# dcharatan/pixelsplat

Measured on NVIDIA H100. Metric: rendered views/sec fwd+bwd @256x256, 3 gauss/px, higher is better.
Workload: dtype f32

## Files before the change

### pixelsplat_b200/csrc/ps_common.cuh

```cuda
#pragma once
#include <cuda_runtime.h>
#include <stdint.h>

#include "../../include/pixelsplat_b200.h"

namespace ps {

constexpr int kTile = PS_TILE;
constexpr int kTilePixels = kTile * kTile;

struct Geom {
    float *depth;
    int32_t *radii;
    float2 *xy;
    float4 *conic_opacity;
    float4 *rgb;
    ushort4 *rect;
    uint8_t *clamped;
    uint32_t *tile_count;
    uint32_t *tile_start;
    uint32_t *tile_cursor;
    long long *n_instances;
    uint32_t *vis_pairs;
    uint32_t *vis_any;
    float4 *cull;
};

struct ImageState {
    float *final_T;
    uint32_t *n_contrib;
    float *color;
    float4 *run_state;
    float *depth_image;
    float *run_depth;
};

constexpr int kLossSlots = PS_LOSS_SLOTS;
struct LossEpilogue {
    const float *target;
    float *sums;
    const float *grad_scale;
};

constexpr int kMaxSegments = 4;

struct HitLists {
    uint2 *hits;
    uint32_t *run_hits;
};

struct Dims {
    int S, V, P, M, deg, sh_layout, cov_layout, H, W, gx, gy, tiles, sh_basis, segK, hit_lists;
    int depth_mode;
    long long capacity;
};

struct Inputs {
    const float *means, *cov, *opac, *sh, *view, *proj, *campos, *tanfov, *bg, *scale;
    const float *near_far;
};

struct ViewGrads {
    float2 *d_mean2d;
    float4 *d_conic;
    float4 *d_color;
};

constexpr float kDepthEps = 1e-10f;

__device__ __forceinline__ float depth_value(int mode, float vz, const float *scale, const float *near_far, int vid) {
    const float z = scale ? vz / scale[vid] : vz;
    if (mode == PS_DEPTH_DISPARITY) return 1.0f / z;
    if (mode == PS_DEPTH_RELATIVE_DISPARITY) {
        const float dn = 1.0f / (near_far[2 * vid] + kDepthEps), df = 1.0f / (near_far[2 * vid + 1] + kDepthEps);
        return 1.0f - (1.0f / (z + kDepthEps) - df) / (dn - df + kDepthEps);
    }
    if (mode == PS_DEPTH_LOG) return logf(fmaxf(fminf(z, near_far[2 * vid]), near_far[2 * vid + 1]));
    return z;
}

__device__ __forceinline__ float depth_value_grad(int mode, float vz, const float *scale, const float *near_far, int vid) {
    const float z = scale ? vz / scale[vid] : vz;
    if (mode == PS_DEPTH_DISPARITY) return -1.0f / (z * z);
    if (mode == PS_DEPTH_RELATIVE_DISPARITY) {
        const float dn = 1.0f / (near_far[2 * vid] + kDepthEps), df = 1.0f / (near_far[2 * vid + 1] + kDepthEps);
        const float iz = 1.0f / (z + kDepthEps);
        return iz * iz / (dn - df + kDepthEps);
    }
    if (mode == PS_DEPTH_LOG) {
        const float nr = near_far[2 * vid], fr = near_far[2 * vid + 1];
        const float m = fminf(z, nr);
        const float gm = z < nr ? 1.0f : (z == nr ? 0.5f : 0.0f);
        const float gr = m > fr ? 1.0f : (m == fr ? 0.5f : 0.0f);
        return gm * gr / fmaxf(m, fr);
    }
    return 1.0f;
}

__device__ __forceinline__ float2 cull_extent(float a, float c, float o) {
    if (!(a > 0.0f) || !(c > 0.0f) || !(o <= 3.0e38f)) return make_float2(3.0e38f, 3.0e38f);
    if (!(o * 255.0f >= 1.0f - 1e-3f)) return make_float2(-3.0e38f, -3.0e38f);
    const float tau2 = 2.0f * (__logf(fmaxf(o * 255.0f, 1.0f)) + 0.01f);
    return make_float2(sqrtf(tau2 * a) * 1.001f + 0.01f, sqrtf(tau2 * c) * 1.001f + 0.01f);
}

void set_error(const char *fmt, ...);

enum Mark { kMarkFwdStart = 0, kMarkPreprocess, kMarkScatter, kMarkSort, kMarkCompositeFwd,
            kMarkBwdStart, kMarkBwdZero, kMarkCompositeBwd, kMarkPreprocessBwd, kNumMarks };
void mark(int id, cudaStream_t st);
void count_launch();

bool first_use_on_device(unsigned long long &mask);

#define PS_CUDA_CHECK(expr)                                                              \
    do {                                                                                 \
        cudaError_t _e = (expr);                                                         \
        if (_e != cudaSuccess) {                                                         \
            ps::set_error("%s failed: %s (%s:%d)", #expr, cudaGetErrorString(_e), __FILE__, __LINE__); \
            return PS_ERR_CUDA;                                                          \
        }                                                                                \
    } while (0)

#define PS_LAUNCH_CHECK(name)                                                            \
    do {                                                                                 \
        cudaError_t _e = cudaGetLastError();                                             \
        if (_e != cudaSuccess) {                                                         \
            ps::set_error("launch of %s failed: %s", name, cudaGetErrorString(_e));      \
            return PS_ERR_CUDA;                                                          \
        }                                                                                \
        ps::count_launch();                                                              \
    } while (0)

int launch_preprocess(const Dims &d, const Inputs &in, const Geom &g, cudaStream_t st);
int launch_sh_color(const Dims &d, const Inputs &in, const Geom &g, cudaStream_t st);
int launch_binning(const Dims &d, const Geom &g, unsigned long long *keys,
                   unsigned long long *keys_alt, int sort_impl, int segment_hint, cudaStream_t st);
int launch_composite_forward(const Dims &d, const Inputs &in, const Geom &g,
                             const unsigned long long *keys, const ImageState &img,
                             float *out_color, const LossEpilogue &loss, const HitLists &hl, cudaStream_t st);
int launch_composite_backward(const Dims &d, const Inputs &in, const Geom &g,
                              const unsigned long long *keys, const ImageState &img,
                              const float *d_color, const float *d_depth, const ViewGrads &vg,
                              const LossEpilogue &loss, const HitLists &hl, cudaStream_t st);
int launch_composite_forward_v1(const Dims &d, const Inputs &in, const Geom &g,
                                const unsigned long long *keys, const ImageState &img,
                                float *out_color, cudaStream_t st);
int launch_composite_backward_v1(const Dims &d, const Inputs &in, const Geom &g,
                                 const unsigned long long *keys, const ImageState &img,
                                 const float *d_color, const ViewGrads &vg, cudaStream_t st);
int composite_impl();
int set_composite_option(int which, int value);
int get_composite_option(int which);
int composite_segments(long long tasks);
bool composite_hit_lists(long long capacity);
int launch_preprocess_backward(const Dims &d, const Inputs &in, const Geom &g, const ViewGrads &vg,
                               const ps_raster_grads &out, cudaStream_t st);
int launch_gradient_fill(const Dims &d, const ps_raster_grads &out, cudaStream_t st);

}
```

### pixelsplat_b200/csrc/raster_api.cu

```cuda
#include <cstdarg>
#include <atomic>
#include <cstdio>
#include <cstring>
#include <mutex>

#include "ps_common.cuh"

namespace ps {

static thread_local char g_error[512] = "";

void set_error(const char *fmt, ...) {
    va_list ap;
    va_start(ap, fmt);
    vsnprintf(g_error, sizeof(g_error), fmt, ap);
    va_end(ap);
}

static bool g_timing = false;
static cudaEvent_t g_events[kNumMarks];
static bool g_events_ready = false;
static std::atomic<unsigned long long> g_launches{0};

void count_launch() { g_launches.fetch_add(1, std::memory_order_relaxed); }

static std::mutex g_once_mutex;

bool first_use_on_device(unsigned long long &mask) {
    int dev = 0;
    cudaGetDevice(&dev);
    const unsigned long long bit = 1ull << (dev & 63);
    std::lock_guard<std::mutex> lock(g_once_mutex);
    if (mask & bit) return false;
    mask |= bit;
    return true;
}

void mark(int id, cudaStream_t st) {
    if (!g_timing) return;
    if (!g_events_ready) {
        for (int i = 0; i < kNumMarks; ++i) cudaEventCreate(&g_events[i]);
        g_events_ready = true;
    }
    cudaEventRecord(g_events[id], st);
}

struct SideCtx {
    cudaStream_t side = nullptr;
    cudaEvent_t fork = nullptr, join = nullptr;
    std::mutex enqueue;
};
static SideCtx g_side_ctx[64];

static int side_ready(SideCtx *&ctx) {
    int dev = 0;
    PS_CUDA_CHECK(cudaGetDevice(&dev));
    ctx = &g_side_ctx[dev & 63];
    std::lock_guard<std::mutex> lock(g_once_mutex);
    if (ctx->side) return PS_OK;
    PS_CUDA_CHECK(cudaStreamCreateWithFlags(&ctx->side, cudaStreamNonBlocking));
    PS_CUDA_CHECK(cudaEventCreateWithFlags(&ctx->fork, cudaEventDisableTiming));
    PS_CUDA_CHECK(cudaEventCreateWithFlags(&ctx->join, cudaEventDisableTiming));
    return PS_OK;
}

static size_t align_up(size_t x) { return (x + 255) & ~(size_t)255; }

struct Layout {
    ps_raster_layout off;
    ps_raster_sizes sizes;
};

static int validate(const ps_raster_desc *d) {
    if (!d) { set_error("desc is NULL"); return PS_ERR_INVALID_ARGUMENT; }
    if (d->n_scenes < 1 || d->views_per_scene < 1 || d->n_gaussians < 1) {
        set_error("n_scenes, views_per_scene and n_gaussians must be >= 1 (got %d, %d, %d)",
                  d->n_scenes, d->views_per_scene, d->n_gaussians);
        return PS_ERR_INVALID_ARGUMENT;
    }
    if (d->height < 1 || d->width < 1) { set_error("bad image size %dx%d", d->height, d->width); return PS_ERR_INVALID_ARGUMENT; }
    if (d->sh_coeffs < 0 || d->sh_coeffs > 25) { set_error("sh_coeffs must be in [0, 25], got %d", d->sh_coeffs); return PS_ERR_INVALID_ARGUMENT; }
    if (d->sh_degree < 0 || d->sh_degree > 4) { set_error("sh_degree must be in [0, 4], got %d", d->sh_degree); return PS_ERR_INVALID_ARGUMENT; }
    if (d->sh_coeffs > 0 && (d->sh_degree + 1) * (d->sh_degree + 1) > d->sh_coeffs) {
        set_error("sh_degree %d needs %d coefficients, only %d given", d->sh_degree,
                  (d->sh_degree + 1) * (d->sh_degree + 1), d->sh_coeffs);
        return PS_ERR_INVALID_ARGUMENT;
    }
    if (d->sh_layout != PS_SH_M3 && d->sh_layout != PS_SH_3M) { set_error("bad sh_layout %d", d->sh_layout); return PS_ERR_INVALID_ARGUMENT; }
    if (d->sh_basis != PS_SH_BASIS_3DGS && d->sh_basis != PS_SH_BASIS_E3NN) { set_error("bad sh_basis %d", d->sh_basis); return PS_ERR_INVALID_ARGUMENT; }
    if (d->depth_mode < PS_DEPTH_NONE || d->depth_mode > PS_DEPTH_LOG) { set_error("bad depth_mode %d (PS_DEPTH_*: 0..4)", d->depth_mode); return PS_ERR_INVALID_ARGUMENT; }
    if (d->cov_layout != PS_COV_TRIU6 && d->cov_layout != PS_COV_3X3) { set_error("bad cov_layout %d", d->cov_layout); return PS_ERR_INVALID_ARGUMENT; }
    if (d->instance_capacity < 1 || d->instance_capacity > 0x7fffffffll) {
        set_error("instance_capacity must be in [1, 2^31-1], got %lld", (long long)d->instance_capacity);
        return PS_ERR_INVALID_ARGUMENT;
    }
    const long long gx = (d->width + kTile - 1) / kTile, gy = (d->height + kTile - 1) / kTile;
    if (gx > 65535 || gy > 65535) { set_error("image too large for 16-bit tile rectangles"); return PS_ERR_UNSUPPORTED; }
    const long long segs = (long long)d->n_scenes * d->views_per_scene * gx * gy;
    if ((long long)d->n_scenes * d->views_per_scene * d->n_gaussians > 0xffffffffll) {
        set_error("scenes * views * gaussians must fit 32 bits");
        return PS_ERR_UNSUPPORTED;
    }
    if (segs > 0x7fffffffll || (long long)d->n_scenes * d->views_per_scene > 65535) {
        set_error("too many (view, tile) segments: %lld", segs);
        return PS_ERR_UNSUPPORTED;
    }
    return PS_OK;
}

static Dims make_dims(const ps_raster_desc *d) {
    Dims r;
    r.S = d->n_scenes; r.V = d->views_per_scene; r.P = d->n_gaussians; r.M = d->sh_coeffs;
    r.deg = d->sh_degree; r.sh_layout = d->sh_layout; r.cov_layout = d->cov_layout;
    r.H = d->height; r.W = d->width;
    r.gx = (d->width + kTile - 1) / kTile; r.gy = (d->height + kTile - 1) / kTile;
    r.tiles = r.gx * r.gy;
    r.capacity = d->instance_capacity;
    r.sh_basis = d->sh_basis;
    r.segK = composite_segments((long long)r.S * r.V * r.tiles * 8);
    r.hit_lists = composite_hit_lists(r.capacity) ? 1 : 0;
    r.depth_mode = d->depth_mode;
    return r;
}

static Layout make_layout(const ps_raster_desc *d) {
    const Dims m = make_dims(d);
    const size_t vp = (size_t)m.S * m.V * m.P;
    const size_t vt = (size_t)m.S * m.V * m.tiles;
    const size_t px = (size_t)m.S * m.V * m.H * m.W;
    Layout L;
    size_t o = 0;
    auto take = [&](size_t bytes) { const size_t at = o; o = align_up(o + bytes); return at; };
    L.off.depth = take(vp * 4);
    L.off.radii = take(vp * 4);
    L.off.xy = take(vp * 8);
    L.off.conic_opacity = take(vp * 16);
    L.off.rgb = take(vp * 16);
    L.off.rect = take(vp * 8);
    L.off.clamped = take(vp);
    L.off.tile_count = take(vt * 4);
    L.off.tile_start = take(vt * 4);
    L.off.tile_cursor = take(vt * 4);
    L.off.n_instances = take(32);
    L.off.vis_pairs = take(vp * 4);
    L.off.vis_any = take((size_t)m.S * m.P * 4);
    L.off.cull = take(vp * 16);
    L.sizes.geom_bytes = o;
    o = 0;
    L.off.keys = take((size_t)m.capacity * 8);
    L.off.keys_alt = take((size_t)m.capacity * 8);
    L.off.block_hits = L.off.run_hits = 0;
    if (m.hit_lists) {
        L.off.block_hits = take((size_t)m.capacity * 8 * 8);
        L.off.run_hits = take((size_t)m.S * m.V * m.tiles * 8 * kMaxSegments * 4);
    }
    L.sizes.binning_bytes = o;
    o = 0;
    L.off.final_T = take(px * 4);
    L.off.n_contrib = take(px * 4);
    L.off.color = take(px * 12);
    L.off.run_state = take(px * 16 * (kMaxSegments - 1));
    L.off.depth_image = L.off.run_depth = 0;
    if (m.depth_mode) {
        L.off.depth_image = take(px * 4);
        L.off.run_depth = take(px * 4 * (kMaxSegments - 1));
    }
    L.sizes.image_bytes = o;
    L.sizes.backward_bytes = align_up(vp * 8) + align_up(vp * 16) + align_up(vp * 16);
    return L;
}

static Geom make_geom(const Layout &L, void *geom) {
    char *b = static_cast<char *>(geom);
    Geom g;
    g.depth = reinterpret_cast<float *>(b + L.off.depth);
    g.radii = reinterpret_cast<int32_t *>(b + L.off.radii);
    g.xy = reinterpret_cast<float2 *>(b + L.off.xy);
    g.conic_opacity = reinterpret_cast<float4 *>(b + L.off.conic_opacity);
    g.rgb = reinterpret_cast<float4 *>(b + L.off.rgb);
    g.rect = reinterpret_cast<ushort4 *>(b + L.off.rect);
    g.clamped = reinterpret_cast<uint8_t *>(b + L.off.clamped);
    g.tile_count = reinterpret_cast<uint32_t *>(b + L.off.tile_count);
    g.tile_start = reinterpret_cast<uint32_t *>(b + L.off.tile_start);
    g.tile_cursor = reinterpret_cast<uint32_t *>(b + L.off.tile_cursor);
    g.n_instances = reinterpret_cast<long long *>(b + L.off.n_instances);
    g.vis_pairs = reinterpret_cast<uint32_t *>(b + L.off.vis_pairs);
    g.vis_any = reinterpret_cast<uint32_t *>(b + L.off.vis_any);
    g.cull = reinterpret_cast<float4 *>(b + L.off.cull);
    return g;
}

static ImageState make_image(const Layout &L, void *image) {
    char *b = static_cast<char *>(image);
    ImageState im;
    im.final_T = reinterpret_cast<float *>(b + L.off.final_T);
    im.n_contrib = reinterpret_cast<uint32_t *>(b + L.off.n_contrib);
    im.color = reinterpret_cast<float *>(b + L.off.color);
    im.run_state = reinterpret_cast<float4 *>(b + L.off.run_state);
    im.depth_image = L.off.depth_image ? reinterpret_cast<float *>(b + L.off.depth_image) : nullptr;
    im.run_depth = L.off.run_depth ? reinterpret_cast<float *>(b + L.off.run_depth) : nullptr;
    return im;
}

static int check_common(const ps_raster_desc *desc, const ps_raster_inputs *in, const ps_raster_state *state,
                        const Layout &L) {
    if (!in || !state) { set_error("inputs/state is NULL"); return PS_ERR_INVALID_ARGUMENT; }
    if (!in->means || !in->cov || !in->opacities || !in->sh || !in->viewmatrix || !in->projmatrix ||
        !in->campos || !in->tanfov || !in->background) {
        set_error("a required input pointer is NULL");
        return PS_ERR_INVALID_ARGUMENT;
    }
    if (!state->geom || !state->binning || !state->image) { set_error("a state buffer is NULL"); return PS_ERR_INVALID_ARGUMENT; }
    if (state->geom_bytes < L.sizes.geom_bytes || state->binning_bytes < L.sizes.binning_bytes ||
        state->image_bytes < L.sizes.image_bytes) {
        set_error("state buffers too small: need geom %zu binning %zu image %zu, got %zu %zu %zu",
                  L.sizes.geom_bytes, L.sizes.binning_bytes, L.sizes.image_bytes, state->geom_bytes,
                  state->binning_bytes, state->image_bytes);
        return PS_ERR_INVALID_ARGUMENT;
    }
    if (((uintptr_t)state->geom | (uintptr_t)state->binning | (uintptr_t)state->image) & 15) {
        set_error("state buffers must be 16-byte aligned");
        return PS_ERR_INVALID_ARGUMENT;
    }
    if ((desc->depth_mode == PS_DEPTH_RELATIVE_DISPARITY || desc->depth_mode == PS_DEPTH_LOG) && !in->near_far) {
        set_error("depth_mode %d needs ps_raster_inputs.near_far", desc->depth_mode);
        return PS_ERR_INVALID_ARGUMENT;
    }
    if (desc->depth_mode && composite_impl() == 1) {
        set_error("the legacy compositor (composite_impl = 1) has no depth channel");
        return PS_ERR_UNSUPPORTED;
    }
    return PS_OK;
}

static Inputs make_inputs(const ps_raster_inputs *in) {
    Inputs r;
    r.means = in->means; r.cov = in->cov; r.opac = in->opacities; r.sh = in->sh;
    r.view = in->viewmatrix; r.proj = in->projmatrix; r.campos = in->campos; r.tanfov = in->tanfov;
    r.bg = in->background; r.scale = in->scene_scale; r.near_far = in->near_far;
    return r;
}

}

using namespace ps;

extern "C" {

PS_API int ps_version(void) { return 100; }

PS_API const char *ps_last_error(void) { return g_error; }

PS_API unsigned long long ps_launch_count(void) { return g_launches.load(std::memory_order_relaxed); }

PS_API void ps_timing_enable(int on) { g_timing = on != 0; }

PS_API int ps_timing_read(float *ms) {
    if (!g_timing || !g_events_ready) { set_error("timing is not enabled"); return PS_ERR_INVALID_ARGUMENT; }
    static const int pairs[7][2] = {{kMarkFwdStart, kMarkPreprocess}, {kMarkPreprocess, kMarkScatter},
                                    {kMarkScatter, kMarkSort}, {kMarkSort, kMarkCompositeFwd},
                                    {kMarkBwdStart, kMarkBwdZero}, {kMarkBwdZero, kMarkCompositeBwd},
                                    {kMarkCompositeBwd, kMarkPreprocessBwd}};
    PS_CUDA_CHECK(cudaEventSynchronize(g_events[kMarkPreprocessBwd]));
    for (int i = 0; i < 7; ++i) PS_CUDA_CHECK(cudaEventElapsedTime(&ms[i], g_events[pairs[i][0]], g_events[pairs[i][1]]));
    return PS_OK;
}

PS_API int ps_set_option(const char *name, int value) {
    if (!name) { set_error("ps_set_option: name is NULL"); return PS_ERR_INVALID_ARGUMENT; }
    int rc = PS_ERR_INVALID_ARGUMENT;
    if (!strcmp(name, "composite_impl")) rc = set_composite_option(0, value);
    else if (!strcmp(name, "composite_segments")) rc = set_composite_option(1, value);
    else if (!strcmp(name, "composite_hit_lists")) rc = set_composite_option(2, value);
    if (rc) set_error("ps_set_option: unknown option or bad value: %s = %d", name, value);
    return rc;
}

PS_API int ps_get_option(const char *name, int *value) {
    if (!name || !value) { set_error("ps_get_option: name / value is NULL"); return PS_ERR_INVALID_ARGUMENT; }
    int which = -1;
    if (!strcmp(name, "composite_impl")) which = 0;
    else if (!strcmp(name, "composite_segments")) which = 1;
    else if (!strcmp(name, "composite_hit_lists")) which = 2;
    if (which < 0) { set_error("ps_get_option: unknown option %s", name); return PS_ERR_INVALID_ARGUMENT; }
    *value = get_composite_option(which);
    return PS_OK;
}

PS_API int ps_raster_sizes_query(const ps_raster_desc *desc, ps_raster_sizes *out) {
    int rc = validate(desc);
    if (rc) return rc;
    if (!out) { set_error("out is NULL"); return PS_ERR_INVALID_ARGUMENT; }
    *out = make_layout(desc).sizes;
    return PS_OK;
}

PS_API int ps_raster_layout_query(const ps_raster_desc *desc, ps_raster_layout *out) {
    int rc = validate(desc);
    if (rc) return rc;
    if (!out) { set_error("out is NULL"); return PS_ERR_INVALID_ARGUMENT; }
    *out = make_layout(desc).off;
    return PS_OK;
}

}

static int raster_forward_impl(const ps_raster_desc *desc, const ps_raster_inputs *in, const ps_raster_state *state,
                               float *out_color, int32_t *out_radii, int64_t *n_instances_host,
                               const ps_raster_loss *loss, void *stream) {
    int rc = validate(desc);
    if (rc) return rc;
    const Layout L = make_layout(desc);
    rc = check_common(desc, in, state, L);
    if (rc) return rc;
    LossEpilogue le{nullptr, nullptr, nullptr};
    if (loss) {
        if (!loss->target || !loss->sums) { set_error("ps_raster_loss: target / sums is NULL"); return PS_ERR_INVALID_ARGUMENT; }
        le.target = loss->target; le.sums = loss->sums;
    } else if (!out_color) {
        set_error("out_color is NULL");
        return PS_ERR_INVALID_ARGUMENT;
    }
    cudaStream_t st = static_cast<cudaStream_t>(stream);
    const Dims d = make_dims(desc);
    const Inputs I = make_inputs(in);
    const Geom g = make_geom(L, state->geom);
    unsigned long long *keys = reinterpret_cast<unsigned long long *>(static_cast<char *>(state->binning) + L.off.keys);
    unsigned long long *keys_alt = reinterpret_cast<unsigned long long *>(static_cast<char *>(state->binning) + L.off.keys_alt);
    const ImageState img = make_image(L, state->image);

    SideCtx *sc = nullptr;
    if ((rc = side_ready(sc))) return rc;
    std::lock_guard<std::mutex> enqueue_lock(sc->enqueue);
    mark(kMarkFwdStart, st);
    if ((rc = launch_preprocess(d, I, g, st))) return rc;
    mark(kMarkPreprocess, st);
    PS_CUDA_CHECK(cudaEventRecord(sc->fork, st));
    PS_CUDA_CHECK(cudaStreamWaitEvent(sc->side, sc->fork, 0));
    if ((rc = launch_sh_color(d, I, g, sc->side))) return rc;
    PS_CUDA_CHECK(cudaEventRecord(sc->join, sc->side));
    if ((rc = launch_binning(d, g, keys, keys_alt, desc->sort_impl, desc->sort_segment_hint, st))) return rc;
    mark(kMarkSort, st);
    PS_CUDA_CHECK(cudaStreamWaitEvent(st, sc->join, 0));
    if (n_instances_host)
        PS_CUDA_CHECK(cudaMemcpyAsync(n_instances_host, g.n_instances, 2 * sizeof(int64_t), cudaMemcpyDeviceToHost, st));
    if (le.sums)
        PS_CUDA_CHECK(cudaMemsetAsync(le.sums, 0, sizeof(float) * 2 * kLossSlots * (size_t)d.S * d.V, st));
    HitLists hl{nullptr, nullptr};
    if (d.hit_lists) {
        hl.hits = reinterpret_cast<uint2 *>(static_cast<char *>(state->binning) + L.off.block_hits);
        hl.run_hits = reinterpret_cast<uint32_t *>(static_cast<char *>(state->binning) + L.off.run_hits);
    }
    if ((rc = launch_composite_forward(d, I, g, keys, img, out_color, le, hl, st))) return rc;
    mark(kMarkCompositeFwd, st);
    if (out_radii)
        PS_CUDA_CHECK(cudaMemcpyAsync(out_radii, g.radii, sizeof(int32_t) * (size_t)d.S * d.V * d.P,
                                      cudaMemcpyDeviceToDevice, st));
    return PS_OK;
}

extern "C" {

PS_API int ps_raster_forward(const ps_raster_desc *desc, const ps_raster_inputs *in, const ps_raster_state *state,
                             float *out_color, int32_t *out_radii, int64_t *n_instances_host, void *stream) {
    return raster_forward_impl(desc, in, state, out_color, out_radii, n_instances_host, nullptr, stream);
}

PS_API int ps_raster_forward_loss(const ps_raster_desc *desc, const ps_raster_inputs *in, const ps_raster_state *state,
                                  const ps_raster_loss *loss, float *out_color, int32_t *out_radii,
                                  int64_t *n_instances_host, void *stream) {
    if (!loss) { set_error("ps_raster_forward_loss: loss is NULL"); return PS_ERR_INVALID_ARGUMENT; }
    return raster_forward_impl(desc, in, state, out_color, out_radii, n_instances_host, loss, stream);
}

}

static int raster_backward_impl(const ps_raster_desc *desc, const ps_raster_inputs *in, const ps_raster_state *state,
                                const float *d_color, const float *target, const float *grad_scale,
                                const float *d_depth, void *scratch, size_t scratch_bytes,
                                const ps_raster_grads *grads, void *stream) {
    int rc = validate(desc);
    if (rc) return rc;
    const Layout L = make_layout(desc);
    rc = check_common(desc, in, state, L);
    if (rc) return rc;
    if ((!d_color && !(target && grad_scale)) || !scratch || !grads) {
        set_error("d_color (or target + grad_scale) / scratch / grads is NULL");
        return PS_ERR_INVALID_ARGUMENT;
    }
    const LossEpilogue le{d_color ? nullptr : target, nullptr, d_color ? nullptr : grad_scale};
    if (!grads->d_means || !grads->d_cov || !grads->d_opacities || !grads->d_sh) {
        set_error("a required gradient pointer is NULL");
        return PS_ERR_INVALID_ARGUMENT;
    }
    if (scratch_bytes < L.sizes.backward_bytes || ((uintptr_t)scratch & 15)) {
        set_error("backward scratch too small or misaligned: need %zu, got %zu", L.sizes.backward_bytes, scratch_bytes);
        return PS_ERR_INVALID_ARGUMENT;
    }
    cudaStream_t st = static_cast<cudaStream_t>(stream);
    Dims d = make_dims(desc);
    if (!d_depth) d.depth_mode = 0;
    const Inputs I = make_inputs(in);
    const Geom g = make_geom(L, state->geom);
    const unsigned long long *keys = reinterpret_cast<const unsigned long long *>(static_cast<char *>(state->binning) + L.off.keys);
    const ImageState img = make_image(L, state->image);
    const size_t vp = (size_t)d.S * d.V * d.P;
    char *sb = static_cast<char *>(scratch);
    ViewGrads vg;
    vg.d_mean2d = reinterpret_cast<float2 *>(sb);
    vg.d_conic = reinterpret_cast<float4 *>(sb + align_up(vp * 8));
    vg.d_color = reinterpret_cast<float4 *>(sb + align_up(vp * 8) + align_up(vp * 16));
    SideCtx *sc = nullptr;
    if ((rc = side_ready(sc))) return rc;
    std::lock_guard<std::mutex> enqueue_lock(sc->enqueue);
    mark(kMarkBwdStart, st);
    PS_CUDA_CHECK(cudaEventRecord(sc->fork, st));
    PS_CUDA_CHECK(cudaStreamWaitEvent(sc->side, sc->fork, 0));
    if ((rc = launch_gradient_fill(d, *grads, sc->side))) return rc;
    PS_CUDA_CHECK(cudaEventRecord(sc->join, sc->side));
    PS_CUDA_CHECK(cudaMemsetAsync(scratch, 0, L.sizes.backward_bytes, st));
    mark(kMarkBwdZero, st);
    HitLists hl{nullptr, nullptr};
    if (d.hit_lists) {
        hl.hits = reinterpret_cast<uint2 *>(static_cast<char *>(state->binning) + L.off.block_hits);
        hl.run_hits = reinterpret_cast<uint32_t *>(static_cast<char *>(state->binning) + L.off.run_hits);
    }
    if ((rc = launch_composite_backward(d, I, g, keys, img, d_color, d_depth, vg, le, hl, st))) return rc;
    mark(kMarkCompositeBwd, st);
    PS_CUDA_CHECK(cudaStreamWaitEvent(st, sc->join, 0));
    if ((rc = launch_preprocess_backward(d, I, g, vg, *grads, st))) return rc;
    mark(kMarkPreprocessBwd, st);
    return PS_OK;
}

extern "C" {

PS_API int ps_raster_backward(const ps_raster_desc *desc, const ps_raster_inputs *in, const ps_raster_state *state,
                              const float *d_color, void *scratch, size_t scratch_bytes,
                              const ps_raster_grads *grads, void *stream) {
    if (!d_color) { set_error("d_color is NULL"); return PS_ERR_INVALID_ARGUMENT; }
    return raster_backward_impl(desc, in, state, d_color, nullptr, nullptr, nullptr, scratch, scratch_bytes, grads,
                                stream);
}

PS_API int ps_raster_backward_loss(const ps_raster_desc *desc, const ps_raster_inputs *in, const ps_raster_state *state,
                                   const float *target, const float *grad_scale, void *scratch, size_t scratch_bytes,
                                   const ps_raster_grads *grads, void *stream) {
    if (!target || !grad_scale) { set_error("target / grad_scale is NULL"); return PS_ERR_INVALID_ARGUMENT; }
    return raster_backward_impl(desc, in, state, nullptr, target, grad_scale, nullptr, scratch, scratch_bytes, grads,
                                stream);
}

PS_API int ps_raster_backward_depth(const ps_raster_desc *desc, const ps_raster_inputs *in, const ps_raster_state *state,
                                    const float *d_color, const float *loss_target, const float *grad_scale,
                                    const float *d_depth, void *scratch, size_t scratch_bytes,
                                    const ps_raster_grads *grads, void *stream) {
    if (!d_depth) { set_error("d_depth is NULL"); return PS_ERR_INVALID_ARGUMENT; }
    if (desc && desc->depth_mode == PS_DEPTH_NONE) {
        set_error("ps_raster_backward_depth needs the depth_mode of a depth forward (got 0)");
        return PS_ERR_INVALID_ARGUMENT;
    }
    if (!d_color && !(loss_target && grad_scale)) { set_error("d_color, or loss_target + grad_scale, is NULL"); return PS_ERR_INVALID_ARGUMENT; }
    return raster_backward_impl(desc, in, state, d_color, d_color ? nullptr : loss_target, d_color ? nullptr : grad_scale,
                                d_depth, scratch, scratch_bytes, grads, stream);
}

}
```

### pixelsplat_b200/csrc/raster_binning.cu

```cuda
#include <cub/device/device_segmented_radix_sort.cuh>

#include "ps_common.cuh"

namespace ps {

constexpr int kScanThreads = 1024;

__global__ void __launch_bounds__(kScanThreads)
k_tile_scan(int n, const uint32_t *__restrict__ count, uint32_t *__restrict__ start,
            uint32_t *__restrict__ cursor, long long *__restrict__ n_instances) {
    __shared__ uint32_t warp_sums[32];
    __shared__ unsigned long long carry_s;
    const int tid = threadIdx.x, lane = tid & 31, warp = tid >> 5;
    if (tid == 0) carry_s = 0;
    __syncthreads();
    uint32_t cmax = 0;
    for (int base = 0; base < n; base += kScanThreads) {
        const int i = base + tid;
        const uint32_t c = i < n ? count[i] : 0u;
        cmax = max(cmax, c);
        uint32_t x = c;
#pragma unroll
        for (int o = 1; o < 32; o <<= 1) {
            const uint32_t y = __shfl_up_sync(0xffffffffu, x, o);
            if (lane >= o) x += y;
        }
        if (lane == 31) warp_sums[warp] = x;
        __syncthreads();
        if (warp == 0) {
            uint32_t w = warp_sums[lane];
#pragma unroll
            for (int o = 1; o < 32; o <<= 1) {
                const uint32_t y = __shfl_up_sync(0xffffffffu, w, o);
                if (lane >= o) w += y;
            }
            warp_sums[lane] = w;
        }
        __syncthreads();
        const unsigned long long carry = carry_s;
        const uint32_t warp_off = warp ? warp_sums[warp - 1] : 0u;
        const unsigned long long excl = carry + warp_off + (x - c);
        if (i < n) {
            const uint32_t e = excl > 0xffffffffull ? 0xffffffffu : (uint32_t)excl;
            start[i] = e;
            cursor[i] = e;
        }
        __syncthreads();
        if (tid == kScanThreads - 1) carry_s = carry + warp_sums[31];
        __syncthreads();
    }
    if (tid == 0) *n_instances = (long long)carry_s;
    cmax = __reduce_max_sync(0xffffffffu, cmax);
    if (lane == 0 && cmax) atomicMax(reinterpret_cast<unsigned long long *>(n_instances + 1), (unsigned long long)cmax);
}

constexpr int kScatterThreads = 256;
constexpr int kScatterMaxSmemTiles = 8192;

__global__ void __launch_bounds__(kScatterThreads)
k_scatter(Dims d, Geom geo, unsigned long long *__restrict__ keys, int use_smem) {
    extern __shared__ uint32_t s_scatter[];
    if (*geo.n_instances > d.capacity) return;
    const int vid = blockIdx.y;
    const int g = blockIdx.x * kScatterThreads + threadIdx.x;
    uint32_t *cnt = s_scatter, *base = s_scatter + d.tiles;
    uint32_t *cur = geo.tile_cursor + (size_t)vid * d.tiles;
    const size_t vg = (size_t)vid * d.P + g;
    const bool vis = g < d.P && geo.radii[vg] > 0;
    ushort4 r = make_ushort4(0, 0, 0, 0);
    unsigned long long key = 0;
    if (vis) {
        r = geo.rect[vg];
        key = ((unsigned long long)__float_as_uint(geo.depth[vg]) << 32) | (uint32_t)g;
    }
    if (!use_smem) {
        for (int ty = r.y; ty < r.w; ++ty)
            for (int tx = r.x; tx < r.z; ++tx) keys[atomicAdd(&cur[ty * d.gx + tx], 1u)] = key;
        return;
    }
    for (int i = threadIdx.x; i < d.tiles; i += kScatterThreads) cnt[i] = 0;
    __syncthreads();
    for (int ty = r.y; ty < r.w; ++ty)
        for (int tx = r.x; tx < r.z; ++tx) atomicAdd(&cnt[ty * d.gx + tx], 1u);
    __syncthreads();
    for (int i = threadIdx.x; i < d.tiles; i += kScatterThreads) {
        const uint32_t c = cnt[i];
        if (c) { base[i] = atomicAdd(&cur[i], c); cnt[i] = 0; }
    }
    __syncthreads();
    for (int ty = r.y; ty < r.w; ++ty)
        for (int tx = r.x; tx < r.z; ++tx) {
            const int t = ty * d.gx + tx;
            keys[base[t] + atomicAdd(&cnt[t], 1u)] = key;
        }
}

template <int THREADS>
__device__ void bitonic_sort_smem(unsigned long long *s_keys, int n_pad) {
    constexpr int kWarps = THREADS / 32;
    const int lane = threadIdx.x & 31, warp = threadIdx.x >> 5;
    const int chunk = max(n_pad / kWarps, 2);
    const int warps_used = n_pad / chunk;
    const int half = n_pad >> 1;
    for (int k = 2; k <= n_pad; k <<= 1) {
        int j = k >> 1;
        const bool had_global = j >= chunk;
        for (; j >= chunk; j >>= 1) {
            for (int t = threadIdx.x; t < half; t += THREADS) {
                const int i = 2 * t - (t & (j - 1));
                const int p = i + j;
                const unsigned long long a = s_keys[i], b = s_keys[p];
                const bool up = (i & k) == 0;
                if ((a > b) == up) { s_keys[i] = b; s_keys[p] = a; }
            }
            __syncthreads();
        }
        if (warp < warps_used) {
            const int base = warp * chunk;
            for (; j > 0; j >>= 1) {
                for (int t = lane; t < (chunk >> 1); t += 32) {
                    const int i = base + 2 * t - (t & (j - 1));
                    const int p = i + j;
                    const unsigned long long a = s_keys[i], b = s_keys[p];
                    const bool up = (i & k) == 0;
                    if ((a > b) == up) { s_keys[i] = b; s_keys[p] = a; }
                }
                __syncwarp();
            }
        }
        if (had_global || 2 * k > chunk) __syncthreads();
    }
}

constexpr int kSortThreads = 512;
constexpr int kSortWarps = kSortThreads / 32;

struct SortSmem {
    uint32_t cnt[kSortWarps * 256];
    uint32_t misc[64];
};

__device__ unsigned long long *radix8_passes(unsigned long long *a, unsigned long long *b, int n, SortSmem &sm,
                                             int key_shift, uint32_t sub, int num_passes) {
    const int tid = threadIdx.x, lane = tid & 31, warp = tid >> 5;
    const int lo = (int)(((long long)n * warp) / kSortWarps);
    const int hi = (int)(((long long)n * (warp + 1)) / kSortWarps);
    uint32_t *cnt = sm.cnt, *misc = sm.misc;
    for (int p = 0; p < num_passes; ++p) {
        const int shift = 8 * p;
        auto digit = [&](unsigned long long k) -> uint32_t {
            return ((((uint32_t)(k >> key_shift)) - sub) >> shift) & 255u;
        };
        for (int i = tid; i < kSortWarps * 256; i += kSortThreads) cnt[i] = 0;
        if (tid == 0) misc[0] = 0;
        __syncthreads();
        for (int i = lo + lane; i < hi; i += 32) atomicAdd(&cnt[warp * 256 + digit(a[i])], 1u);
        __syncthreads();
        uint32_t total = 0, incl = 0;
        if (tid < 256) {
            uint32_t c[kSortWarps];
#pragma unroll
            for (int w = 0; w < kSortWarps; ++w) c[w] = cnt[w * 256 + tid];
#pragma unroll
            for (int w = 0; w < kSortWarps; ++w) { const uint32_t t = c[w]; c[w] = total; total += t; }
            if (total == (uint32_t)n) misc[0] = 1;
            incl = total;
#pragma unroll
            for (int o = 1; o < 32; o <<= 1) {
                const uint32_t y = __shfl_up_sync(0xffffffffu, incl, o);
                if (lane >= o) incl += y;
            }
            if (lane == 31) misc[8 + warp] = incl;
#pragma unroll
            for (int w = 0; w < kSortWarps; ++w) cnt[w * 256 + tid] = c[w];
        }
        __syncthreads();
        if (misc[0]) { __syncthreads(); continue; }
        if (tid < 256) {
            uint32_t off = incl - total;
            for (int w = 0; w < warp; ++w) off += misc[8 + w];
#pragma unroll
            for (int w = 0; w < kSortWarps; ++w) cnt[w * 256 + tid] += off;
        }
        __syncthreads();
        for (int base = lo; base < hi; base += 32) {
            const int i = base + lane;
            const bool valid = i < hi;
            const unsigned long long key = valid ? a[i] : 0ull;
            const uint32_t dg = valid ? digit(key) : (256u + (uint32_t)lane);
            const uint32_t peers = __match_any_sync(0xffffffffu, dg);
            const int leader = __ffs(peers) - 1;
            const int rank = __popc(peers & ((1u << lane) - 1u));
            uint32_t off = 0;
            if (valid && lane == leader) {
                off = cnt[warp * 256 + dg];
                cnt[warp * 256 + dg] = off + (uint32_t)__popc(peers);
            }
            off = __shfl_sync(0xffffffffu, off, leader);
            if (valid) b[off + rank] = key;
            __syncwarp();
        }
        __syncthreads();
        unsigned long long *t = a; a = b; b = t;
    }
    return a;
}

static size_t sort_smem_bytes(int cap) { return sizeof(SortSmem) + sizeof(unsigned long long) * 2 * (size_t)cap; }

__global__ void __launch_bounds__(kSortThreads)
k_tile_sort(const uint32_t *__restrict__ tile_start, const uint32_t *__restrict__ tile_count,
            const long long *__restrict__ n_instances, long long capacity,
            unsigned long long *__restrict__ keys, unsigned long long *__restrict__ keys_alt, int cap, int id_bits) {
    extern __shared__ __align__(16) unsigned char s_sort[];
    if (*n_instances > capacity) return;
    const int seg = blockIdx.x;
    const int n = (int)tile_count[seg];
    if (n < 2) return;
    const uint32_t s0 = tile_start[seg];
    SortSmem &sm = *reinterpret_cast<SortSmem *>(s_sort);
    const int tid = threadIdx.x, lane = tid & 31;
    if (n > cap) {
        unsigned long long *r = radix8_passes(keys + s0, keys_alt + s0, n, sm, 0, 0u, (id_bits + 7) / 8);
        unsigned long long *o = (r == keys + s0) ? keys_alt + s0 : keys + s0;
        r = radix8_passes(r, o, n, sm, 32, 0u, 4);
        if (r != keys + s0)
            for (int i = tid; i < n; i += kSortThreads) keys[s0 + i] = r[i];
        return;
    }
    unsigned long long *A = reinterpret_cast<unsigned long long *>(s_sort + sizeof(SortSmem));
    unsigned long long *B = A + cap;
    if (tid == 0) { sm.misc[1] = 0xffffffffu; sm.misc[2] = 0u; sm.misc[3] = 0u; }
    __syncthreads();
    uint32_t dlo = 0xffffffffu, dhi = 0u;
    for (int i = tid; i < n; i += kSortThreads) {
        const unsigned long long k = keys[s0 + i];
        A[i] = k;
        const uint32_t dpt = (uint32_t)(k >> 32);
        dlo = min(dlo, dpt); dhi = max(dhi, dpt);
    }
    dlo = __reduce_min_sync(0xffffffffu, dlo);
    dhi = __reduce_max_sync(0xffffffffu, dhi);
    if (lane == 0) { atomicMin(&sm.misc[1], dlo); atomicMax(&sm.misc[2], dhi); }
    __syncthreads();
    const uint32_t dmin = sm.misc[1], range = sm.misc[2] - dmin;
    const int bits = range ? 32 - __clz(range) : 0;
    __syncthreads();
    A = radix8_passes(A, B, n, sm, 32, dmin, (bits + 7) / 8);
    for (int i = tid; i < n; i += kSortThreads) {
        const uint32_t dpt = (uint32_t)(A[i] >> 32);
        const bool starts = (i == 0 || (uint32_t)(A[i - 1] >> 32) != dpt) && (i + 1 < n) &&
                            (uint32_t)(A[i + 1] >> 32) == dpt;
        if (starts) {
            int e = i + 2;
            while (e < n && (uint32_t)(A[e] >> 32) == dpt) ++e;
            if (e - i > 64) {
                sm.misc[3] = 1u;
            } else {
                for (int x = i + 1; x < e; ++x) {
                    const unsigned long long v = A[x];
                    int y = x - 1;
                    while (y >= i && A[y] > v) { A[y + 1] = A[y]; --y; }
                    A[y + 1] = v;
                }
            }
        }
    }
    __syncthreads();
    if (sm.misc[3]) {
        int n_pad = 2;
        while (n_pad < n) n_pad <<= 1;
        for (int i = n + tid; i < n_pad; i += kSortThreads) A[i] = ~0ull;
        __syncthreads();
        bitonic_sort_smem<kSortThreads>(A, n_pad);
    }
    for (int i = tid; i < n; i += kSortThreads) keys[s0 + i] = A[i];
}

int launch_binning(const Dims &d, const Geom &g, unsigned long long *keys,
                   unsigned long long *keys_alt, int sort_impl, int segment_hint, cudaStream_t st) {
    const int n_seg = d.S * d.V * d.tiles;
    k_tile_scan<<<1, kScanThreads, 0, st>>>(n_seg, g.tile_count, g.tile_start, g.tile_cursor, g.n_instances);
    PS_LAUNCH_CHECK("k_tile_scan");
    const int use_smem = d.tiles <= kScatterMaxSmemTiles;
    static unsigned long long scatter_attr_devices = 0;
    if (first_use_on_device(scatter_attr_devices)) {
        PS_CUDA_CHECK(cudaFuncSetAttribute(k_scatter, cudaFuncAttributeMaxDynamicSharedMemorySize,
                                           (int)(2 * sizeof(uint32_t) * kScatterMaxSmemTiles)));
    }
    dim3 sgrid((d.P + kScatterThreads - 1) / kScatterThreads, d.S * d.V);
    k_scatter<<<sgrid, kScatterThreads, use_smem ? 2 * sizeof(uint32_t) * d.tiles : 0, st>>>(d, g, keys, use_smem);
    PS_LAUNCH_CHECK("k_scatter");
    mark(kMarkScatter, st);

    int id_bits = 1;
    while ((1ll << id_bits) < d.P) ++id_bits;

    if (sort_impl == 1) {
        size_t temp = 0;
        cub::DoubleBuffer<unsigned long long> db(keys, keys_alt);
        PS_CUDA_CHECK(cub::DeviceSegmentedRadixSort::SortKeys(nullptr, temp, db, (int)d.capacity, n_seg,
                                                              g.tile_start, g.tile_cursor, 0, 64, st));
        void *tmp = nullptr;
        PS_CUDA_CHECK(cudaMallocAsync(&tmp, temp, st));
        PS_CUDA_CHECK(cub::DeviceSegmentedRadixSort::SortKeys(tmp, temp, db, (int)d.capacity, n_seg,
                                                              g.tile_start, g.tile_cursor, 0, 64, st));
        if (db.Current() != keys)
            PS_CUDA_CHECK(cudaMemcpyAsync(keys, db.Current(), sizeof(unsigned long long) * (size_t)d.capacity,
                                          cudaMemcpyDeviceToDevice, st));
        PS_CUDA_CHECK(cudaFreeAsync(tmp, st));
        return PS_OK;
    }

    int cap = 2048;
    if (segment_hint > 0) {
        const long long want = (long long)segment_hint + segment_hint / 4;
        while (cap < want && cap < 8192) cap <<= 1;
    }
    static unsigned long long battr_devices = 0;
    if (first_use_on_device(battr_devices)) {
        PS_CUDA_CHECK(cudaFuncSetAttribute(k_tile_sort, cudaFuncAttributeMaxDynamicSharedMemorySize,
                                           (int)sort_smem_bytes(8192)));
    }
    k_tile_sort<<<n_seg, kSortThreads, sort_smem_bytes(cap), st>>>(
        g.tile_start, g.tile_count, g.n_instances, d.capacity, keys, keys_alt, cap, id_bits);
    PS_LAUNCH_CHECK("k_tile_sort");
    return PS_OK;
}

}
```

### pixelsplat_b200/csrc/raster_preprocess.cu

```cuda
#include "ps_common.cuh"
#include "raster_math.cuh"

namespace ps {

constexpr int kPreThreads = 128;

__device__ __forceinline__ void warp_append(bool flag, uint32_t value, uint32_t *list, long long *counter, int lane) {
    const unsigned m = __ballot_sync(0xffffffffu, flag);
    if (m == 0u) return;
    const int leader = __ffs(m) - 1;
    unsigned long long base = 0;
    if (lane == leader)
        base = atomicAdd(reinterpret_cast<unsigned long long *>(counter), (unsigned long long)__popc(m));
    base = __shfl_sync(0xffffffffu, base, leader);
    if (flag) list[base + __popc(m & ((1u << lane) - 1u))] = value;
}

__global__ void __launch_bounds__(kPreThreads)
k_preprocess(Dims d, Inputs in, Geom geo, int use_smem_hist) {
    extern __shared__ uint32_t s_hist[];
    const int hist_n = d.V * d.tiles;
    const int scene = blockIdx.y;
    const int lane = threadIdx.x & 31;
    const int g = blockIdx.x * kPreThreads + threadIdx.x;
    const bool live = g < d.P;
    if (use_smem_hist) {
        for (int i = threadIdx.x; i < hist_n; i += kPreThreads) s_hist[i] = 0;
        __syncthreads();
    }
    const size_t sg = (size_t)scene * d.P + (live ? g : 0);
    float mx0 = 0.0f, my0 = 0.0f, mz0 = 0.0f, opacity = 0.0f;
    if (live) {
        mx0 = in.means[3 * sg + 0]; my0 = in.means[3 * sg + 1]; mz0 = in.means[3 * sg + 2];
        opacity = in.opac[sg];
    }
    const float *covp = in.cov + sg * (d.cov_layout == PS_COV_TRIU6 ? 6 : 9);
    float cov_raw[6];
    {
        float tmp[6] = {0.0f, 0.0f, 0.0f, 0.0f, 0.0f, 0.0f};
        if (live) load_cov6(covp, d.cov_layout, 1.0f, tmp);
#pragma unroll
        for (int i = 0; i < 6; ++i) cov_raw[i] = tmp[i];
    }
    bool any_vis = false;

    for (int v = 0; v < d.V; ++v) {
        const int vid = scene * d.V + v;
        const size_t vg = (size_t)vid * d.P + (live ? g : 0);
        const float *__restrict__ vm = in.view + 16 * vid;
        const float *__restrict__ pm = in.proj + 16 * vid;
        const float sc = in.scale ? in.scale[vid] : 1.0f;
        const float px = in.scale ? mx0 * sc : mx0;
        const float py = in.scale ? my0 * sc : my0;
        const float pz = in.scale ? mz0 * sc : mz0;
        bool vis = live;
        float vz = 0.0f;
        if (vis) {
            geo.radii[vg] = 0;
            vz = vm[2] * px + vm[6] * py + vm[10] * pz + vm[14];
            vis = !(vz <= 0.2f);
        }
        if (vis) {
            const float hx = pm[0] * px + pm[4] * py + pm[8] * pz + pm[12];
            const float hy = pm[1] * px + pm[5] * py + pm[9] * pz + pm[13];
            const float hw = pm[3] * px + pm[7] * py + pm[11] * pz + pm[15];
            const float p_w = 1.0f / (hw + 0.0000001f);
            const float projx = hx * p_w, projy = hy * p_w;
            const float tanfovx = in.tanfov[2 * vid], tanfovy = in.tanfov[2 * vid + 1];
            const float focal_x = (float)d.W / (2.0f * tanfovx);
            const float focal_y = (float)d.H / (2.0f * tanfovy);
            float s6[6];
            {
                const float sc2 = sc * sc;
#pragma unroll
                for (int i = 0; i < 6; ++i) s6[i] = in.scale ? cov_raw[i] * sc2 : cov_raw[i];
            }
            Cov2D cv;
            compute_cov2d(px, py, pz, s6, vm, focal_x, focal_y, tanfovx, tanfovy, cv);
            const float det = cv.a * cv.c - cv.b * cv.b;
            vis = !(det == 0.0f);
            if (vis) {
                const float det_inv = 1.0f / det;
                const float mid = 0.5f * (cv.a + cv.c);
                const float sq = sqrtf(fmaxf(0.1f, mid * mid - det));
                const float lambda1 = mid + sq, lambda2 = mid - sq;
                const float my_radius = ceilf(3.0f * sqrtf(fmaxf(lambda1, lambda2)));
                const float pixx = ((projx + 1.0f) * (float)d.W - 1.0f) * 0.5f;
                const float pixy = ((projy + 1.0f) * (float)d.H - 1.0f) * 0.5f;
                const int r = (int)my_radius;
                const float rf = (float)r;
                const int minx = min(d.gx, max(0, (int)((pixx - rf) / (float)kTile)));
                const int miny = min(d.gy, max(0, (int)((pixy - rf) / (float)kTile)));
                const int maxx = min(d.gx, max(0, (int)((pixx + rf + (float)(kTile - 1)) / (float)kTile)));
                const int maxy = min(d.gy, max(0, (int)((pixy + rf + (float)(kTile - 1)) / (float)kTile)));
                vis = (maxx - minx) * (maxy - miny) != 0;
                if (vis) {
                    geo.depth[vg] = vz;
                    geo.radii[vg] = r;
                    geo.xy[vg] = make_float2(pixx, pixy);
                    geo.conic_opacity[vg] = make_float4(cv.c * det_inv, -cv.b * det_inv, cv.a * det_inv, opacity);
                    {
                        const float2 ext = cull_extent(cv.a, cv.c, opacity);
                        geo.cull[vg] = make_float4(pixx, pixy, ext.x, ext.y);
                    }
                    geo.rect[vg] = make_ushort4((unsigned short)minx, (unsigned short)miny,
                                                (unsigned short)maxx, (unsigned short)maxy);
                    if (d.M == 0) {
                        const float *__restrict__ col = in.sh + sg * 3;
                        const float dv = d.depth_mode ? depth_value(d.depth_mode, vz, in.scale, in.near_far, vid) : 0.0f;
                        geo.rgb[vg] = make_float4(col[0], col[1], col[2], dv);
                        geo.clamped[vg] = 0;
                    }
                    for (int ty = miny; ty < maxy; ++ty)
                        for (int tx = minx; tx < maxx; ++tx) {
                            const int t = ty * d.gx + tx;
                            if (use_smem_hist) atomicAdd(&s_hist[v * d.tiles + t], 1u);
                            else atomicAdd(&geo.tile_count[(size_t)vid * d.tiles + t], 1u);
                        }
                }
            }
        }
        any_vis |= vis;
        warp_append(vis, (uint32_t)vg, geo.vis_pairs, geo.n_instances + 2, lane);
    }
    warp_append(any_vis, (uint32_t)sg, geo.vis_any, geo.n_instances + 3, lane);
    if (use_smem_hist) {
        __syncthreads();
        uint32_t *dst = geo.tile_count + (size_t)scene * d.V * d.tiles;
        for (int i = threadIdx.x; i < hist_n; i += kPreThreads) {
            const uint32_t c = s_hist[i];
            if (c) atomicAdd(&dst[i], c);
        }
    }
}

constexpr int kShThreads = 128;

__global__ void __launch_bounds__(kShThreads)
k_sh_color(Dims d, Inputs in, Geom geo, int row_stride) {
    extern __shared__ float s_rows[];
    const long long n = geo.n_instances[2];
    const int lane = threadIdx.x & 31, warp = threadIdx.x >> 5;
    const long long i0 = ((long long)blockIdx.x * kShThreads) + warp * 32;
    if (i0 >= n) return;
    const long long i = i0 + lane;
    const bool live = i < n;
    const uint32_t vg = live ? geo.vis_pairs[i] : 0u;
    const uint32_t vid = vg / (uint32_t)d.P, g = vg - vid * (uint32_t)d.P;
    const uint32_t scene = vid / (uint32_t)d.V;
    const size_t sg = (size_t)scene * d.P + g;
    const int sh_n = 3 * d.M;
    float *wrows = s_rows + (size_t)warp * 32 * row_stride;
    gather_rows_async(in.sh, (unsigned long long)sg, (int)min((long long)32, n - i0), sh_n, wrows, row_stride, lane);
    const float sc = in.scale ? in.scale[vid] : 1.0f;
    const float m0 = in.means[3 * sg + 0], m1 = in.means[3 * sg + 1], m2 = in.means[3 * sg + 2];
    const float px = in.scale ? m0 * sc : m0, py = in.scale ? m1 * sc : m1, pz = in.scale ? m2 * sc : m2;
    const float cx = in.campos[3 * vid], cy = in.campos[3 * vid + 1], cz = in.campos[3 * vid + 2];
    const float ddx = px - cx, ddy = py - cy, ddz = pz - cz;
    const float len = sqrtf(ddx * ddx + ddy * ddy + ddz * ddz);
    const float x = ddx / len, y = ddy / len, z = ddz / len;
    gather_rows_wait();
    if (!live) return;
    const float *row = wrows + lane * row_stride;
    float acc[3] = {0.0f, 0.0f, 0.0f};
    const int M = d.M, layout = d.sh_layout;
    const float3 sa = sh_arg(d.sh_basis, x, y, z);
    const uint32_t flip = sh_flip_mask(d.sh_basis);
    sh_for_each(d.deg, sa.x, sa.y, sa.z, [&](int k, float Yk, float, float, float) {
        const float Y = sh_sign(flip, k, Yk);
#pragma unroll
        for (int ch = 0; ch < 3; ++ch) {
            const float c = row[sh_index(layout, M, k, ch)];
            acc[ch] = k == 0 ? Y * c : acc[ch] + Y * c;
        }
    });
    float rgb[3];
    uint8_t clamp_bits = 0;
#pragma unroll
    for (int ch = 0; ch < 3; ++ch) {
        const float a = acc[ch] + 0.5f;
        if (a < 0.0f) clamp_bits |= (uint8_t)(1u << ch);
        rgb[ch] = fmaxf(a, 0.0f);
    }
    const float dv = d.depth_mode ? depth_value(d.depth_mode, geo.depth[vg], in.scale, in.near_far, (int)vid) : 0.0f;
    geo.rgb[vg] = make_float4(rgb[0], rgb[1], rgb[2], dv);
    geo.clamped[vg] = clamp_bits;
}

int launch_sh_color(const Dims &d, const Inputs &in, const Geom &g, cudaStream_t st) {
    if (d.M == 0) return PS_OK;
    const int row_stride = (3 * d.M) | 1;
    const size_t smem = sizeof(float) * kShThreads * row_stride;
    static unsigned long long attr_devices = 0;
    if (first_use_on_device(attr_devices)) {
        PS_CUDA_CHECK(cudaFuncSetAttribute(k_sh_color, cudaFuncAttributeMaxDynamicSharedMemorySize, 64 * 1024));
    }
    const long long pairs = (long long)d.S * d.V * d.P;
    k_sh_color<<<(unsigned)((pairs + kShThreads - 1) / kShThreads), kShThreads, smem, st>>>(d, in, g, row_stride);
    PS_LAUNCH_CHECK("k_sh_color");
    return PS_OK;
}

int launch_preprocess(const Dims &d, const Inputs &in, const Geom &g, cudaStream_t st) {
    PS_CUDA_CHECK(cudaMemsetAsync(g.tile_count, 0, sizeof(uint32_t) * (size_t)d.S * d.V * d.tiles, st));
    PS_CUDA_CHECK(cudaMemsetAsync(g.n_instances, 0, 4 * sizeof(long long), st));
    const size_t hist_bytes = sizeof(uint32_t) * (size_t)d.V * d.tiles;
    const int use_smem = hist_bytes <= 32 * 1024;
    dim3 grid((d.P + kPreThreads - 1) / kPreThreads, d.S);
    k_preprocess<<<grid, kPreThreads, use_smem ? hist_bytes : 0, st>>>(d, in, g, use_smem);
    PS_LAUNCH_CHECK("k_preprocess");
    return PS_OK;
}

}
```

Baseline: 2733.

## Fuse tile scan into preprocess via last-block pattern and drop extra copies

The standalone single-block tile-count scan kernel is removed. Its work now runs in the last CTA to finish k_preprocess, detected with an atomic counter and threadfences. Radii are written straight to the output buffer, which removes a D2D memcpy. The instance counts go to mapped host memory when it is available, which removes a D2H memcpy, and the two memsets are merged into one contiguous memset. This cuts kernel launches and copies per forward pass, at the cost of a serial scan tail on a single CTA of preprocess-sized threads and a reliance on contiguous buffer layout for the merged memset.

```diff
diff --git a/pixelsplat_b200/csrc/ps_common.cuh b/pixelsplat_b200/csrc/ps_common.cuh
--- a/pixelsplat_b200/csrc/ps_common.cuh
+++ b/pixelsplat_b200/csrc/ps_common.cuh
@@ -25,6 +25,7 @@
     uint32_t *vis_any;
     float4 *cull;
 };
+constexpr int kInstanceSlots = 5;
 
 struct ImageState {
     float *final_T;
@@ -132,7 +133,8 @@
         ps::count_launch();                                                              \
     } while (0)
 
-int launch_preprocess(const Dims &d, const Inputs &in, const Geom &g, cudaStream_t st);
+int launch_preprocess(const Dims &d, const Inputs &in, const Geom &g, int32_t *out_radii, long long *n_host,
+                      cudaStream_t st);
 int launch_sh_color(const Dims &d, const Inputs &in, const Geom &g, cudaStream_t st);
 int launch_binning(const Dims &d, const Geom &g, unsigned long long *keys,
                    unsigned long long *keys_alt, int sort_impl, int segment_hint, cudaStream_t st);
diff --git a/pixelsplat_b200/csrc/raster_api.cu b/pixelsplat_b200/csrc/raster_api.cu
--- a/pixelsplat_b200/csrc/raster_api.cu
+++ b/pixelsplat_b200/csrc/raster_api.cu
@@ -141,7 +141,7 @@
     L.off.tile_count = take(vt * 4);
     L.off.tile_start = take(vt * 4);
     L.off.tile_cursor = take(vt * 4);
-    L.off.n_instances = take(32);
+    L.off.n_instances = take(kInstanceSlots * sizeof(long long));
     L.off.vis_pairs = take(vp * 4);
     L.off.vis_any = take((size_t)m.S * m.P * 4);
     L.off.cull = take(vp * 16);
@@ -332,8 +332,16 @@
     SideCtx *sc = nullptr;
     if ((rc = side_ready(sc))) return rc;
     std::lock_guard<std::mutex> enqueue_lock(sc->enqueue);
+    long long *n_host_dev = nullptr;
+    if (n_instances_host) {
+        cudaPointerAttributes pa;
+        if (cudaPointerGetAttributes(&pa, n_instances_host) != cudaSuccess)
+            cudaGetLastError();
+        else if (pa.type == cudaMemoryTypeHost)
+            n_host_dev = static_cast<long long *>(pa.devicePointer);
+    }
     mark(kMarkFwdStart, st);
-    if ((rc = launch_preprocess(d, I, g, st))) return rc;
+    if ((rc = launch_preprocess(d, I, g, out_radii, n_host_dev, st))) return rc;
     mark(kMarkPreprocess, st);
     PS_CUDA_CHECK(cudaEventRecord(sc->fork, st));
     PS_CUDA_CHECK(cudaStreamWaitEvent(sc->side, sc->fork, 0));
@@ -342,7 +350,7 @@
     if ((rc = launch_binning(d, g, keys, keys_alt, desc->sort_impl, desc->sort_segment_hint, st))) return rc;
     mark(kMarkSort, st);
     PS_CUDA_CHECK(cudaStreamWaitEvent(st, sc->join, 0));
-    if (n_instances_host)
+    if (n_instances_host && !n_host_dev)
         PS_CUDA_CHECK(cudaMemcpyAsync(n_instances_host, g.n_instances, 2 * sizeof(int64_t), cudaMemcpyDeviceToHost, st));
     if (le.sums)
         PS_CUDA_CHECK(cudaMemsetAsync(le.sums, 0, sizeof(float) * 2 * kLossSlots * (size_t)d.S * d.V, st));
@@ -353,9 +361,6 @@
     }
     if ((rc = launch_composite_forward(d, I, g, keys, img, out_color, le, hl, st))) return rc;
     mark(kMarkCompositeFwd, st);
-    if (out_radii)
-        PS_CUDA_CHECK(cudaMemcpyAsync(out_radii, g.radii, sizeof(int32_t) * (size_t)d.S * d.V * d.P,
-                                      cudaMemcpyDeviceToDevice, st));
     return PS_OK;
 }
 
diff --git a/pixelsplat_b200/csrc/raster_binning.cu b/pixelsplat_b200/csrc/raster_binning.cu
--- a/pixelsplat_b200/csrc/raster_binning.cu
+++ b/pixelsplat_b200/csrc/raster_binning.cu
@@ -3,56 +3,6 @@
 #include "ps_common.cuh"
 
 namespace ps {
-
-constexpr int kScanThreads = 1024;
-
-__global__ void __launch_bounds__(kScanThreads)
-k_tile_scan(int n, const uint32_t *__restrict__ count, uint32_t *__restrict__ start,
-            uint32_t *__restrict__ cursor, long long *__restrict__ n_instances) {
-    __shared__ uint32_t warp_sums[32];
-    __shared__ unsigned long long carry_s;
-    const int tid = threadIdx.x, lane = tid & 31, warp = tid >> 5;
-    if (tid == 0) carry_s = 0;
-    __syncthreads();
-    uint32_t cmax = 0;
-    for (int base = 0; base < n; base += kScanThreads) {
-        const int i = base + tid;
-        const uint32_t c = i < n ? count[i] : 0u;
-        cmax = max(cmax, c);
-        uint32_t x = c;
-#pragma unroll
-        for (int o = 1; o < 32; o <<= 1) {
-            const uint32_t y = __shfl_up_sync(0xffffffffu, x, o);
-            if (lane >= o) x += y;
-        }
-        if (lane == 31) warp_sums[warp] = x;
-        __syncthreads();
-        if (warp == 0) {
-            uint32_t w = warp_sums[lane];
-#pragma unroll
-            for (int o = 1; o < 32; o <<= 1) {
-                const uint32_t y = __shfl_up_sync(0xffffffffu, w, o);
-                if (lane >= o) w += y;
-            }
-            warp_sums[lane] = w;
-        }
-        __syncthreads();
-        const unsigned long long carry = carry_s;
-        const uint32_t warp_off = warp ? warp_sums[warp - 1] : 0u;
-        const unsigned long long excl = carry + warp_off + (x - c);
-        if (i < n) {
-            const uint32_t e = excl > 0xffffffffull ? 0xffffffffu : (uint32_t)excl;
-            start[i] = e;
-            cursor[i] = e;
-        }
-        __syncthreads();
-        if (tid == kScanThreads - 1) carry_s = carry + warp_sums[31];
-        __syncthreads();
-    }
-    if (tid == 0) *n_instances = (long long)carry_s;
-    cmax = __reduce_max_sync(0xffffffffu, cmax);
-    if (lane == 0 && cmax) atomicMax(reinterpret_cast<unsigned long long *>(n_instances + 1), (unsigned long long)cmax);
-}
 
 constexpr int kScatterThreads = 256;
 constexpr int kScatterMaxSmemTiles = 8192;
@@ -280,8 +230,6 @@
 int launch_binning(const Dims &d, const Geom &g, unsigned long long *keys,
                    unsigned long long *keys_alt, int sort_impl, int segment_hint, cudaStream_t st) {
     const int n_seg = d.S * d.V * d.tiles;
-    k_tile_scan<<<1, kScanThreads, 0, st>>>(n_seg, g.tile_count, g.tile_start, g.tile_cursor, g.n_instances);
-    PS_LAUNCH_CHECK("k_tile_scan");
     const int use_smem = d.tiles <= kScatterMaxSmemTiles;
     static unsigned long long scatter_attr_devices = 0;
     if (first_use_on_device(scatter_attr_devices)) {
diff --git a/pixelsplat_b200/csrc/raster_preprocess.cu b/pixelsplat_b200/csrc/raster_preprocess.cu
--- a/pixelsplat_b200/csrc/raster_preprocess.cu
+++ b/pixelsplat_b200/csrc/raster_preprocess.cu
@@ -16,8 +16,69 @@
     if (flag) list[base + __popc(m & ((1u << lane) - 1u))] = value;
 }
 
+constexpr int kScanPerThread = 8;
+
+__device__ void tile_scan_cta(int n, const uint32_t *count, uint32_t *start, uint32_t *cursor,
+                              long long *n_instances, long long *n_host) {
+    constexpr int kWarps = kPreThreads / 32;
+    constexpr int kRound = kPreThreads * kScanPerThread;
+    __shared__ uint32_t warp_sums[kWarps];
+    __shared__ unsigned long long carry_s;
+    __shared__ uint32_t cmax_s;
+    const int tid = threadIdx.x, lane = tid & 31, warp = tid >> 5;
+    if (tid == 0) { carry_s = 0; cmax_s = 0; }
+    __syncthreads();
+    uint32_t cmax = 0;
+    for (int base = 0; base < n; base += kRound) {
+        const int i0 = base + tid * kScanPerThread;
+        uint32_t c[kScanPerThread];
+        uint32_t own = 0;
+#pragma unroll
+        for (int j = 0; j < kScanPerThread; ++j) {
+            c[j] = i0 + j < n ? __ldcg(count + i0 + j) : 0u;
+            cmax = max(cmax, c[j]);
+            own += c[j];
+        }
+        uint32_t x = own;
+#pragma unroll
+        for (int o = 1; o < 32; o <<= 1) {
+            const uint32_t y = __shfl_up_sync(0xffffffffu, x, o);
+            if (lane >= o) x += y;
+        }
+        if (lane == 31) warp_sums[warp] = x;
+        __syncthreads();
+        uint32_t warp_off = 0, block_sum = 0;
+#pragma unroll
+        for (int w = 0; w < kWarps; ++w) {
+            if (w < warp) warp_off += warp_sums[w];
+            block_sum += warp_sums[w];
+        }
+        unsigned long long excl = carry_s + warp_off + (x - own);
+#pragma unroll
+        for (int j = 0; j < kScanPerThread; ++j) {
+            if (i0 + j < n) {
+                const uint32_t e = excl > 0xffffffffull ? 0xffffffffu : (uint32_t)excl;
+                start[i0 + j] = e;
+                cursor[i0 + j] = e;
+            }
+            excl += c[j];
+        }
+        __syncthreads();
+        if (tid == 0) carry_s += block_sum;
+        __syncthreads();
+    }
+    cmax = __reduce_max_sync(0xffffffffu, cmax);
+    if (lane == 0) atomicMax(&cmax_s, cmax);
+    __syncthreads();
+    if (tid == 0) {
+        n_instances[0] = (long long)carry_s;
+        n_instances[1] = (long long)cmax_s;
+        if (n_host) { n_host[0] = (long long)carry_s; n_host[1] = (long long)cmax_s; }
+    }
+}
+
 __global__ void __launch_bounds__(kPreThreads)
-k_preprocess(Dims d, Inputs in, Geom geo, int use_smem_hist) {
+k_preprocess(Dims d, Inputs in, Geom geo, int use_smem_hist, int32_t *out_radii, long long *n_host) {
     extern __shared__ uint32_t s_hist[];
     const int hist_n = d.V * d.tiles;
     const int scene = blockIdx.y;
@@ -57,6 +118,7 @@
         float vz = 0.0f;
         if (vis) {
             geo.radii[vg] = 0;
+            if (out_radii) out_radii[vg] = 0;
             vz = vm[2] * px + vm[6] * py + vm[10] * pz + vm[14];
             vis = !(vz <= 0.2f);
         }
@@ -97,6 +159,7 @@
                 if (vis) {
                     geo.depth[vg] = vz;
                     geo.radii[vg] = r;
+                    if (out_radii) out_radii[vg] = r;
                     geo.xy[vg] = make_float2(pixx, pixy);
                     geo.conic_opacity[vg] = make_float4(cv.c * det_inv, -cv.b * det_inv, cv.a * det_inv, opacity);
                     {
@@ -132,6 +195,17 @@
             if (c) atomicAdd(&dst[i], c);
         }
     }
+    __shared__ bool s_last;
+    __threadfence();
+    __syncthreads();
+    if (threadIdx.x == 0) {
+        const unsigned long long ctas = (unsigned long long)gridDim.x * gridDim.y;
+        s_last = atomicAdd(reinterpret_cast<unsigned long long *>(geo.n_instances + 4), 1ull) == ctas - 1;
+    }
+    __syncthreads();
+    if (!s_last) return;
+    __threadfence();
+    tile_scan_cta(d.S * d.V * d.tiles, geo.tile_count, geo.tile_start, geo.tile_cursor, geo.n_instances, n_host);
 }
 
 constexpr int kShThreads = 128;
@@ -201,13 +275,14 @@
     return PS_OK;
 }
 
-int launch_preprocess(const Dims &d, const Inputs &in, const Geom &g, cudaStream_t st) {
-    PS_CUDA_CHECK(cudaMemsetAsync(g.tile_count, 0, sizeof(uint32_t) * (size_t)d.S * d.V * d.tiles, st));
-    PS_CUDA_CHECK(cudaMemsetAsync(g.n_instances, 0, 4 * sizeof(long long), st));
+int launch_preprocess(const Dims &d, const Inputs &in, const Geom &g, int32_t *out_radii, long long *n_host,
+                      cudaStream_t st) {
+    const size_t zero_bytes = reinterpret_cast<char *>(g.n_instances + kInstanceSlots) - reinterpret_cast<char *>(g.tile_count);
+    PS_CUDA_CHECK(cudaMemsetAsync(g.tile_count, 0, zero_bytes, st));
     const size_t hist_bytes = sizeof(uint32_t) * (size_t)d.V * d.tiles;
     const int use_smem = hist_bytes <= 32 * 1024;
     dim3 grid((d.P + kPreThreads - 1) / kPreThreads, d.S);
-    k_preprocess<<<grid, kPreThreads, use_smem ? hist_bytes : 0, st>>>(d, in, g, use_smem);
+    k_preprocess<<<grid, kPreThreads, use_smem ? hist_bytes : 0, st>>>(d, in, g, use_smem, out_radii, n_host);
     PS_LAUNCH_CHECK("k_preprocess");
     return PS_OK;
 }
```

Result: faster. 2836, median of 6 (+3.8%).
